# Janspiry/Image-Super-Resolution-via-Iterative-Refinement

Hardware: AMD Instinct MI355X
Metric: SR3 16->128 images/sec (2000-step sample) (higher is better)
Workload: dtype f32 via 3xbf16 split MFMA; 1 GPU; SR3 16->128 UNet (reference config/sr_sr3_16_128.json; BASELINE.json configs[1]), batch 16 per GPU, 2000-step p_sample_loop via hipGraph replay; step = one reverse step of the batch; images/s = n_gpus*batch/(2000*t_step); batch_per_gpu=16, global_batch=16, image_size=128, params=97807491, parallelism=independent batches per rank (no collective), weights=random init (PyTorch default, seed 0), output_finite=True

## Files before the change

image-super-resolution-via-iterative-refinement_amd/csrc/abi_ops.hip:

```cpp
#include "plan_internal.h"
#include "tile_code.h"

namespace {

enum Derive { DERIVE_IGEMM_WSPLIT, DERIVE_WINO, DERIVE_WINO_SPLIT };
size_t derive_bytes(const ConvParams& c, Derive kind) {
  const int Cin = c.C0 + c.C1;
  return (kind == DERIVE_IGEMM_WSPLIT ? igemm_wsplit_floats(c.Cout, c.ksize * c.ksize, Cin) : wino_weight_floats(c.Cout, Cin, kind == DERIVE_WINO_SPLIT)) * sizeof(float);
}
int derive_behind_slabs(const ConvParams& c, int tile, int ksplit, Derive kind, void* scratch, size_t* scratch_bytes, hipStream_t st, float** out) {
  const size_t slab = conv_splitk_bytes(c, tile, ksplit);
  const size_t need = derive_bytes(c, kind);
  if (!scratch || *scratch_bytes < slab + need) {
    set_error("conv: %s (%zu < %zu)", kind == DERIVE_IGEMM_WSPLIT ? "scratch too small for the pre-split weights" : "Winograd scratch too small", *scratch_bytes, slab + need);
    return SR3_E_NOMEM;
  }
  *out = reinterpret_cast<float*>(static_cast<char*>(scratch) + slab);
  *scratch_bytes = slab;
  const int Cin = c.C0 + c.C1;
  return kind == DERIVE_IGEMM_WSPLIT ? igemm_split_weights(c.w, c.Cout, c.ksize * c.ksize, Cin, *out, st)
                                     : wino_transform_weights(c.w, c.Cout, Cin, *out, st, kind == DERIVE_WINO_SPLIT);
}

int check_scratch_aligned(const void* scratch) {
// ... 205 lines not shown
  return attention_forward(qkv, B, N, C, out, static_cast<hipStream_t>(stream));
}
int sr3_attention_ex_f32(const float* qkv, int B, int N, int C, float* out, int split, void* stream) {
  if (!qkv || !out) { set_error("null argument"); return SR3_E_BADARG; }
  return attention_forward(qkv, B, N, C, out, static_cast<hipStream_t>(stream), split);
}
int sr3_film_embed_f32(int variant, int B, int inner, const float* level, const int64_t* timestep, const float* freq,
                       const float* w1, const float* b1, const float* w2, const float* b2, const float* wf,
                       const float* bf, int F, float* temb_scratch, float* film_out, void* stream) {
  EmbedParams e;
  memset(&e, 0, sizeof(e));
  e.variant = variant; e.B = B; e.inner = inner; e.level = level; e.tstep = timestep; e.freq = freq;
  e.w1 = w1; e.b1 = b1; e.w2 = w2; e.b2 = b2; e.wf = wf; e.bf = bf; e.F = F; e.temb = temb_scratch; e.film = film_out;
  return embed_forward(e, static_cast<hipStream_t>(stream));
}
int sr3_conv_in_f32(const float* a, int Ca, const float* b, int Cb, int B, int H, int W, const float* w,
                    const float* bias, int Cout, float* out, void* stream) {
  return conv_in_nchw(a, Ca, b, b ? Cb : 0, B, H, W, w, bias, Cout, out, nullptr, static_cast<hipStream_t>(stream));
}
int sr3_conv_out_f32(const float* x, const float* ss, int B, int H, int W, int C, const float* w, const float* bias,
                     int Cout, float* out, void* stream) {
  return conv_out_nchw(x, ss, B, H, W, C, w, bias, Cout, out, static_cast<hipStream_t>(stream));
}

}
```

image-super-resolution-via-iterative-refinement_amd/csrc/plan_abi.hip:

```cpp
#include <stdarg.h>
#include <stdlib.h>
#include <stdio.h>
#include <string.h>

#include <new>
#include <vector>

#include "plan_internal.h"
#include "tile_code.h"

namespace sr3 {

static thread_local char g_err[512] = "";
void set_error(const char* fmt, ...) {
  va_list ap;
  va_start(ap, fmt);
  vsnprintf(g_err, sizeof(g_err), fmt, ap);
  va_end(ap);
}
int hip_fail(hipError_t e, const char* what) {
  set_error("HIP error %d (%s) at %s", (int)e, hipGetErrorString(e), what);
  (void)hipGetLastError();
  return (int)e > 0 ? (int)e : 1;
}
const char* last_error() { return g_err; }

}

int check_store_wt(const sr3_plan*, const char*, int value) {
  if (value < 0 || value > STORE_WT_ALL) { set_error("store_wt %d: a mask of bits 0-2 (0 .. %d)", value, (int)STORE_WT_ALL); return SR3_E_BADARG; }
  return SR3_OK;
}
int check_gemm_epi(const sr3_plan*, const char*, int value) {
  if (value < 0 || value > 2) { set_error("gemm_epi %d: 0 (4-byte epilogue), 1 (16-byte stores) or 2 (16-byte stores written through L2)", value); return SR3_E_BADARG; }
  return SR3_OK;
}
int check_var_channels(const sr3_plan* plan, const char*, int value) {
  if (value != 0 && value * 2 != plan->out_ch) {
    set_error("var_channels %d: 0 or half of out_channel %d (the variance head of a learned-variance model)", value, plan->out_ch);
    return SR3_E_BADARG;
  }
  return SR3_OK;
}
// ... 316 lines not shown
```

image-super-resolution-via-iterative-refinement_amd/csrc/plan_internal.h:

```cpp
#pragma once
#include <map>
#include <string>
#include <vector>

#include "../../include/sr3_mi355x.h"
#include "sr3_common.h"

namespace sr3 {

struct Tensor {
  size_t off = 0;
  size_t bytes = 0;
  int C = 0, H = 0, W = 0;
  size_t stat_off = 0;
  int stat_T = 0;
  bool stats_done = false;
  bool valid = false;
};

struct ResLayer {
  std::string name;
  int cin, cout, skip;
  bool attn;
  int film_off;
// ... 137 lines not shown
  int wgrad_split = 1;
  int attn_split = 1;
  int attn_long = 0;
  int attn_heads = 1;
  int attn_head_dim = 0;
  int gemm_tile = 0;
  int gemm_split = 1;
  int gemm_wpre = 0;
  int fold_fuse = 1;
  int gemm2 = 1;
  int gemm_s2 = 1;
  int gemm_n64 = 1;
  int wino_ragged = 1;
  int wino_up = 1;
  int store_wt = 3;
  int gemm_epi = GEMM_EPI_DEFAULT;
  bool gemm_epi_named = false;
  int launch_gemm_epi() const { return gemm_epi_named ? gemm_epi : -1; }
  int train_geom = 0;
  int fork_side = 0;
  int loss_l2 = 0;
};

enum OptionEffect {
  OPT_FORWARD = 1,
  OPT_TRAIN = 2,
  OPT_REBUILD = OPT_FORWARD | OPT_TRAIN,
  OPT_STALE = 4,
  OPT_RELAY = 8,
  OPT_EXPERIMENT = 16,
};
typedef int (*OptionCheck)(const sr3_plan* plan, const char* key, int value);
int check_store_wt(const sr3_plan*, const char*, int);
int check_gemm_epi(const sr3_plan*, const char*, int);
int check_var_channels(const sr3_plan*, const char*, int);
int check_attn_heads(const sr3_plan*, const char*, int);
struct OptionRow { const char* name; int PlanOptions::*slot; unsigned effects; OptionCheck check; };
static const OptionRow PLAN_OPTIONS[] = {
  {"fuse_stats", &PlanOptions::fuse_stats, OPT_REBUILD, nullptr},
  {"tile_cfg", &PlanOptions::tile_cfg, OPT_REBUILD | OPT_STALE, nullptr},
  {"ksplit", &PlanOptions::ksplit, OPT_REBUILD, nullptr},
  {"keep_all", &PlanOptions::keep_all, OPT_REBUILD, nullptr},
  {"fuse_res", &PlanOptions::fuse_res, OPT_REBUILD, nullptr},
  {"split_bf16", &PlanOptions::split_bf16, OPT_REBUILD | OPT_STALE | OPT_EXPERIMENT, nullptr},
  {"winograd", &PlanOptions::winograd, OPT_REBUILD | OPT_STALE, nullptr},
  {"wino_split", &PlanOptions::wino_split, OPT_REBUILD | OPT_RELAY, nullptr},
  {"wino_split8", &PlanOptions::wino_split8, OPT_REBUILD, nullptr},
  {"wgrad_split", &PlanOptions::wgrad_split, 0, nullptr},
  {"attn_split", &PlanOptions::attn_split, 0, nullptr},
  {"store_wt", &PlanOptions::store_wt, 0, check_store_wt},
  {"gemm_epi", &PlanOptions::gemm_epi, 0, check_gemm_epi},
  {"attn_long", &PlanOptions::attn_long, OPT_REBUILD, nullptr},
  {"gemm_split", &PlanOptions::gemm_split, OPT_REBUILD | OPT_RELAY, nullptr},
  {"gemm_wpre", &PlanOptions::gemm_wpre, OPT_REBUILD | OPT_RELAY, nullptr},
  {"gemm2", &PlanOptions::gemm2, OPT_REBUILD | OPT_RELAY, nullptr},
  {"gemm_s2", &PlanOptions::gemm_s2, OPT_REBUILD | OPT_RELAY, nullptr},
  {"fork_side", &PlanOptions::fork_side, OPT_REBUILD, nullptr},
  {"gemm_n64", &PlanOptions::gemm_n64, OPT_REBUILD | OPT_RELAY, nullptr},
  {"fold_fuse", &PlanOptions::fold_fuse, OPT_REBUILD, nullptr},
  {"gemm_tile", &PlanOptions::gemm_tile, OPT_REBUILD, nullptr},
  {"wino2", &PlanOptions::wino2, OPT_REBUILD, nullptr},
  {"wino_ragged", &PlanOptions::wino_ragged, OPT_REBUILD, nullptr},
  {"wino_up", &PlanOptions::wino_up, OPT_REBUILD, nullptr},
  {"train_geom", &PlanOptions::train_geom, OPT_REBUILD, nullptr},
  {"loss_l2", &PlanOptions::loss_l2, 0, nullptr},
  {"var_channels", &PlanOptions::var_channels, OPT_REBUILD, check_var_channels},
// ... 99 lines not shown
```

image-super-resolution-via-iterative-refinement_amd/csrc/plan_run.hip:

```cpp
#include <string.h>

#include <vector>

#include "plan_internal.h"
#include "tile_code.h"

namespace sr3 {

template <typename T> static T* bind(char* base, size_t off) { return off == NO_OFF ? nullptr : reinterpret_cast<T*>(base + off); }
static const float* bind(const float* params, size_t off) { return off == NO_OFF ? nullptr : params + off; }

struct Bound {
  sr3_plan* P;
  const ForwardCall& f;
  const Regions& R;
  char* ws; char* stats; float* film;
  const float* params;
  hipStream_t st = nullptr;
  hipEvent_t mid = nullptr;
};

static FoldTail make_fold_tail(const FoldSpec& s, const Bound& b) {
  FoldTail f;
  memset(&f, 0, sizeof(f));
// ... 28 lines not shown
  }
  return SR3_OK;
}

static int launch_embed(const Op&, const Bound& b) {
  const sr3_plan* P = b.P;
  const ForwardCall& f = b.f;
  EmbedParams e;
  memset(&e, 0, sizeof(e));
  e.variant = P->d.variant; e.B = f.batch; e.inner = P->d.inner_channel;
  e.level = f.level; e.tstep = f.tstep; e.level_table = f.level_table; e.step_dev = f.step_dev; e.t_map = f.t_map; e.freq = f.freq;
  e.step_out = f.fuse ? const_cast<int*>(f.fuse->step_cur) : nullptr;
  e.w1 = b.params + P->emb_w1; e.b1 = b.params + P->emb_b1; e.w2 = b.params + P->emb_w2; e.b2 = b.params + P->emb_b2;
  e.wf = b.params + P->film_w; e.bf = b.params + P->film_b; e.F = P->film_rows();
  e.temb = reinterpret_cast<float*>(b.ws + b.R.temb_off); e.film = b.film;
  return embed_forward(e, b.st);
}

static int launch_conv_in(const Op& o, const Bound& b) {
  const Op::ConvIn& v = o.conv_in;
  const ForwardCall& f = b.f;
  const float* a0 = f.cond_channels > 0 ? f.cond : f.x;
  const int Ca = f.cond_channels > 0 ? f.cond_channels : v.x_channels;
  const float* a1 = f.cond_channels > 0 ? f.x : nullptr;
  const int Cb = f.cond_channels > 0 ? v.x_channels : 0;
  return conv_in_nchw(a0, Ca, a1, Cb, f.batch, v.H, v.W, b.params + v.w, b.params + v.bias, v.Cout, bind<float>(b.ws, v.out),
                      bind<double>(b.stats, v.ostat), b.st);
}

static int launch_stats(const Op& o, const Bound& b) {
  const Op::Stats& v = o.stats;
  if (o.fold_fused) {
    FoldTail ft = make_fold_tail(o.tail, b);
    return chan_stats_fold(bind<const float>(b.ws, v.src), b.f.batch, v.pixels, v.channels, bind<double>(b.stats, v.stat), ft, b.st);
  }
  return chan_stats(bind<const float>(b.ws, v.src), b.f.batch, v.pixels, v.channels, bind<double>(b.stats, v.stat), b.st);
}

static int launch_fold(const Op& o, const Bound& b) {
  const Op::Fold& v = o.fold;
  return gn_finalize(bind<const double>(b.stats, v.stat0), v.C0, v.T0, bind<const double>(b.stats, v.stat1), v.C1, v.T1, b.f.batch, v.pixels,
                     b.P->d.norm_groups, b.params + v.gamma, b.params + v.beta, 1e-5f, bind<float>(b.ws, b.R.ss_off + o.ss_rel), b.st,
// ... 31 lines not shown
  FoldTail ft;
  if (o.fold_fused) { ft = make_fold_tail(o.tail, b); c.fold = &ft; }
  return conv_forward(c, ch.tile_cfg, ch.ksplit, bind<float>(b.ws, b.R.scratch_off), b.R.scratch_bytes, b.st, b.mid);
}

static int launch_attn(const Op& o, const Bound& b) {
  const Op::Attn& v = o.attn;
  return attention_forward_heads(bind<const float>(b.ws, v.qkv), b.f.batch, v.tokens, v.channels, v.heads, bind<float>(b.ws, v.out), b.st,
                                 (b.P->opt.attn_split ? 1 : 0) | (v.tile_cfg == 24 ? 2 : 0));
}

static int launch_conv_out(const Op& o, const Bound& b) {
  const Op::ConvOut& v = o.conv_out;
  const int rows = (b.f.train || b.f.full_out) ? v.out_ch : v.out_ch - b.P->opt.var_channels;
  return conv_out_nchw(bind<const float>(b.ws, v.src), bind<const float>(b.ws, b.R.ss_off + o.ss_rel), b.f.batch, v.H, v.W, v.channels,
                       b.params + v.w, b.params + v.bias, rows, b.f.eps_out, b.st, b.f.fuse);
}

static int fork_op(sr3_plan* P, const Op& o, hipStream_t main_st, hipStream_t* st) {
  *st = main_st;
  if (o.wait_id >= 0 && o.wait_id < (int)P->join_ev.size()) SR3_HIP(hipStreamWaitEvent(main_st, P->join_ev[o.wait_id], 0));
  if (o.side_id < 0) return SR3_OK;
  if (!P->side_stream) SR3_HIP(hipStreamCreateWithFlags(&P->side_stream, hipStreamNonBlocking));
  while ((int)P->fork_ev.size() <= o.side_id) {
    hipEvent_t a, b;
    SR3_HIP(hipEventCreateWithFlags(&a, hipEventDisableTiming));
    SR3_HIP(hipEventCreateWithFlags(&b, hipEventDisableTiming));
    P->fork_ev.push_back(a); P->join_ev.push_back(b);
  }
  SR3_HIP(hipEventRecord(P->fork_ev[o.side_id], main_st));
  SR3_HIP(hipStreamWaitEvent(P->side_stream, P->fork_ev[o.side_id], 0));
// ... 90 lines not shown
```

image-super-resolution-via-iterative-refinement_amd/csrc/small_kernels.hip:

```cpp
#include <string.h>

#include <type_traits>

#include "conv_prologue.h"
#include "step_tail.h"

namespace sr3 {

__global__ __launch_bounds__(256) void k_chan_stats(const float* __restrict__ x, int HW, int C, int LQ,
                                                     int pix_per_block, double* __restrict__ stat) {
  __shared__ double red[256 * 8];
  const int tid = threadIdx.x;
  const int nq = C >> 2;
  const int ql = tid % LQ, pl = tid / LQ, PP = 256 / LQ;
  const int q = blockIdx.y * LQ + ql;
  const int b = blockIdx.z;
  const int T = gridDim.x;
  const int p0 = blockIdx.x * pix_per_block;
  const int p1 = min(HW, p0 + pix_per_block);
  double s[4] = {0, 0, 0, 0}, s2[4] = {0, 0, 0, 0};
  if (q < nq) {
    const float* base = x + (size_t)b * HW * C + q * 4;
    for (int p = p0 + pl; p < p1; p += PP) {
      const f32x4 v = *reinterpret_cast<const f32x4*>(base + (size_t)p * C);
// ... 428 lines not shown
    }
    const int co0 = cobase + cog * 16;
#pragma unroll
    for (int e4 = 0; e4 < 4; ++e4) {
      const int co = co0 + e4 * 4;
      if (co < Cout) {
        f32x4 o;
#pragma unroll
        for (int e = 0; e < 4; ++e) o[e] = acc[e4 * 4 + e] + (bias ? bias[co + e] : 0.f);
        *reinterpret_cast<f32x4*>(out + (size_t)m * Cout + co) = o;
      }
    }
  }
}

template <int CIN, int NB>
__global__ __launch_bounds__(256) void k_conv_in_mfma(const float* __restrict__ a, int Ca, const float* __restrict__ bsrc,
                                                       int Cb, int B, int H, int W, const float* __restrict__ w,
                                                       const float* __restrict__ bias, float* __restrict__ out,
                                                       double* __restrict__ ostat, int bpw, int T) {
  constexpr int K = 9 * CIN, KS = (K + 1) / 2, Cout = 32 * NB;
  const int lane = threadIdx.x & 63, wave = threadIdx.x >> 6;
  const int ln = lane & 31, h = lane >> 5;
  const int HW = H * W, bpi = HW >> 5;
  const int task = blockIdx.x * 4 + wave;
  if (task >= B * (bpi / bpw)) return;
  const int blk0 = task * bpw;
  const int b = blk0 / bpi;
  const int slice = (blk0 - b * bpi) / bpw;

  float bw[KS][NB], bn[NB];
#pragma unroll
  for (int s = 0; s < KS; ++s)
#pragma unroll
    for (int nb = 0; nb < NB; ++nb) {
      const int k = 2 * s + h;
      bw[s][nb] = k < K ? w[(size_t)(nb * 32 + ln) * K + k] : 0.f;
    }
#pragma unroll
  for (int nb = 0; nb < NB; ++nb) bn[nb] = bias ? bias[nb * 32 + ln] : 0.f;

  const float* plane[CIN];
#pragma unroll
  for (int c = 0; c < CIN; ++c)
    plane[c] = c < Ca ? a + ((size_t)b * Ca + c) * HW : bsrc + ((size_t)b * Cb + (c - Ca)) * HW;

  auto load_block = [&](int blk, float (&av)[KS]) {
    const int p0 = (blk - b * bpi) * 32;
    const int oh = p0 / W, ow = p0 - oh * W + ln;
    const int pixoff = oh * W + ow;
    const bool up = oh > 0, down = oh < H - 1, left = ow > 0, right = ow < W - 1;
#pragma unroll
// ... 65 lines not shown
static constexpr bool CONV_IN7_NB[5] = {false, true, true, true, true};
#endif
static int conv_in_bpw(int Cin, int H, int W, int Cout) {
  if ((Cin != 3 && Cin != 6 && Cin != 7 && Cin != 9) || (W & 31) || (Cout & 31) || Cout > 128 || Cout < 32) return 0;
  if (Cin == 9 && !CONV_IN9_NB[Cout / 32]) return 0;
  if (Cin == 7 && !CONV_IN7_NB[Cout / 32]) return 0;
  const int bpi = H * W / 32;
  return (bpi % 4 == 0) ? 4 : 1;
}
int conv_in_stat_slices(int Cin, int H, int W, int Cout) {
  const int bpw = conv_in_bpw(Cin, H, W, Cout);
  return bpw ? H * W / 32 / bpw : 0;
}

int conv_in_nchw(const float* a, int Ca, const float* b, int Cb, int B, int H, int W, const float* w,
                 const float* bias, int Cout, float* out, double* ostat, hipStream_t st) {
  if (const int bpw = conv_in_bpw(Ca + Cb, H, W, Cout)) {
    const int T = H * W / 32 / bpw;
    const long tasks = (long)B * T;
    const dim3 grid((unsigned)((tasks + 3) / 4));
#define SR3_CI(CIN, NB) hipLaunchKernelGGL((k_conv_in_mfma<CIN, NB>), grid, dim3(256), 0, st, a, Ca, b, Cb, B, H, W, w, bias, out, ostat, bpw, T)
#define SR3_CI_NB(CIN) do { if (nb == 1) SR3_CI(CIN, 1); else if (nb == 2) SR3_CI(CIN, 2); else if (nb == 3) SR3_CI(CIN, 3); else SR3_CI(CIN, 4); } while (0)
    const int nb = Cout / 32;
    switch (Ca + Cb) {
      case 3: SR3_CI_NB(3); break;
      case 6: SR3_CI_NB(6); break;
      case 7: SR3_CI_NB(7); break;
      default: SR3_CI_NB(9); break;
    }
#undef SR3_CI_NB
#undef SR3_CI
    SR3_LAUNCH_CHECK("k_conv_in_mfma");
    return SR3_OK;
  }
  if (ostat) { set_error("conv_in: fused output statistics need the MFMA form (W %% 32 == 0, Cout %% 32 == 0, 3, 6, 7 or 9 input channels)"); return SR3_E_UNSUPPORTED; }
  if (Cout & 3) { set_error("conv_in: Cout %% 4 != 0"); return SR3_E_UNSUPPORTED; }
  const int CoutP = (Cout + 63) & ~63;
  const size_t smem = (size_t)9 * (Ca + Cb) * CoutP * sizeof(float);
  if (smem > 64 * 1024) { set_error("conv_in: weights do not fit LDS (%zu B)", smem); return SR3_E_UNSUPPORTED; }
  const long M = (long)B * H * W;
  hipLaunchKernelGGL(k_conv_in_nchw, dim3((unsigned)((M + 63) / 64)), dim3(256), smem, st, a, Ca, b, Cb, B, H, W, w,
                     bias, Cout, out);
  SR3_LAUNCH_CHECK("k_conv_in_nchw");
  return SR3_OK;
}

#ifdef SR3_CONV_OUT_LINES
constexpr int OT_H = 8, OT_W = 32, OT_CK = 32, OT_LD = 36;
#else
constexpr int OT_H = 8, OT_W = 32, OT_CK = 16, OT_LD = 20;
#endif
constexpr int OT_Q = OT_CK / 4, OT_SUB = OT_CK / 16;
template <int COUT, bool FULL, bool FUSE, bool HIST>
__global__ __launch_bounds__(256) void k_conv_out_nchw(const float* __restrict__ x, const float* __restrict__ ss,
                                                        int B, int H, int W, int C, const float* __restrict__ w,
                                                        const float* __restrict__ bias, int Cout,
                                                        float* __restrict__ out, const StepFuse f) {
  __shared__ f32x4 tile_v[(OT_H + 2) * (OT_W + 2) * OT_LD / 4];
  float* tile = reinterpret_cast<float*>(tile_v);
  const int tid = threadIdx.x;
  const int tx = tid & 31, ty = tid >> 5;
  const int tiles_w = (W + OT_W - 1) / OT_W, tiles_h = (H + OT_H - 1) / OT_H;
  int bid = blockIdx.x;
  const int b = bid / (tiles_w * tiles_h);
  bid -= b * tiles_w * tiles_h;
  const int th = bid / tiles_w, tw = bid - th * tiles_w;
  const int h0 = th * OT_H, w0 = tw * OT_W;
  float acc[COUT <= 4 ? 4 : COUT] = {};
  constexpr int NPIX = (OT_H + 2) * (OT_W + 2);
  for (int c0 = 0; c0 < C; c0 += OT_CK) {
    __syncthreads();
    for (int i = tid; i < NPIX * OT_Q; i += 256) {
      const int pix = i / OT_Q, q = i % OT_Q;
      const int py = pix / (OT_W + 2), px = pix - py * (OT_W + 2);
      const int ih = h0 + py - 1, iw = w0 + px - 1;
      const int c = c0 + q * 4;
      f32x4 v = {0.f, 0.f, 0.f, 0.f};
      if (c < C && (unsigned)ih < (unsigned)H && (unsigned)iw < (unsigned)W) {
        v = *reinterpret_cast<const f32x4*>(x + (((size_t)b * H + ih) * W + iw) * C + c);
        const float* s = ss + ((size_t)b * C + c) * 2;
#pragma unroll
        for (int e = 0; e < 4; ++e) v[e] = silu_libm(fmaf(v[e], s[2 * e], s[2 * e + 1]));
      }
      *reinterpret_cast<f32x4*>(tile + pix * OT_LD + q * 4) = v;
    }
    __syncthreads();
#pragma unroll
    for (int sub = 0; sub < OT_SUB; ++sub) {
#pragma unroll
      for (int tap = 0; tap < 9; ++tap) {
        const float* tp = tile + ((ty + tap / 3) * (OT_W + 2) + tx + tap % 3) * OT_LD + sub * 16;
#pragma unroll
        for (int q = 0; q < 4; ++q) {
          if (FULL || c0 + sub * 16 + q * 4 < C) {
            const f32x4 v = *reinterpret_cast<const f32x4*>(tp + q * 4);
#pragma unroll
            for (int co = 0; co < COUT; ++co) {
              const float* wr = w + ((size_t)co * 9 + tap) * C + c0 + sub * 16 + q * 4;
              acc[co] = fmaf(v[0], wr[0], acc[co]);
              acc[co] = fmaf(v[1], wr[1], acc[co]);
              acc[co] = fmaf(v[2], wr[2], acc[co]);
// ... 17 lines not shown
      const size_t idx = (((size_t)b * Cout + co) * H + oh) * W + ow;
      const float e = acc[co] + (bias ? bias[co] : 0.f);
      if (!FUSE || out) out[idx] = e;
      if (FUSE) {
        const float xv = f.x[idx], zv = f.z ? f.z[idx] : 0.f;
        float hv = HIST ? f.hist[idx] : 0.f;
        const float xn = step_tail<HIST>(cf, f.clip, xv, e, zv, hv);
        if (HIST) f.hist[idx] = hv;
        f.x[idx] = xn;
      }
    }
  }
}

int conv_out_nchw(const float* x, const float* ss, int B, int H, int W, int C, const float* w, const float* bias,
                  int Cout, float* out_nchw, hipStream_t st, const StepFuse* fuse) {
  const bool wide = Cout == 6 || Cout == 8;
  if ((Cout > 4 && !wide) || Cout < 1) { set_error("conv_out: Cout %d > 4 unsupported", Cout); return SR3_E_UNSUPPORTED; }
  if (wide && fuse) { set_error("conv_out: no fused step tail on Cout %d (launch the prediction rows alone)", Cout); return SR3_E_UNSUPPORTED; }
  if (C & 3) { set_error("conv_out: C %% 4 != 0"); return SR3_E_UNSUPPORTED; }
  if (!fuse && !out_nchw) { set_error("conv_out: null output"); return SR3_E_BADARG; }
  const int tiles = ((W + OT_W - 1) / OT_W) * ((H + OT_H - 1) / OT_H) * B;
  StepFuse f;
  memset(&f, 0, sizeof(f));
  if (fuse) f = *fuse;
  if (const int rc = check_step_history("conv_out", f.c3, f.hist, f.x, out_nchw, (size_t)B * Cout * H * W * sizeof(float))) return rc;
  const bool hist = fuse && fuse->hist;
#define SR3_CO_LAUNCH3(N, FU, FS, HI)                                                                                        \
  hipLaunchKernelGGL((k_conv_out_nchw<N, FU, FS, HI>), dim3(tiles), dim3(256), 0, st, x, ss, B, H, W, C, w, bias, Cout, out_nchw, f);
#define SR3_CO_LAUNCH2(N, FU)                                                                                                \
  if (hist) { SR3_CO_LAUNCH3(N, FU, true, true) } else if (fuse) { SR3_CO_LAUNCH3(N, FU, true, false) } else { SR3_CO_LAUNCH3(N, FU, false, false) }
#define SR3_CO_LAUNCH(N)                                                                                                    \
  {                                                                                                                          \
    if (C % OT_CK == 0) { SR3_CO_LAUNCH2(N, true) } else { SR3_CO_LAUNCH2(N, false) }                                       \
  }
  switch (Cout) {
    case 1: SR3_CO_LAUNCH(1) break;
    case 2: SR3_CO_LAUNCH(2) break;
    case 3: SR3_CO_LAUNCH(3) break;
    case 4: SR3_CO_LAUNCH(4) break;
    case 6: if (C % OT_CK == 0) { SR3_CO_LAUNCH3(6, true, false, false) } else { SR3_CO_LAUNCH3(6, false, false, false) } break;
    default: if (C % OT_CK == 0) { SR3_CO_LAUNCH3(8, true, false, false) } else { SR3_CO_LAUNCH3(8, false, false, false) } break;
  }
#undef SR3_CO_LAUNCH
#undef SR3_CO_LAUNCH2
#undef SR3_CO_LAUNCH3
  SR3_LAUNCH_CHECK("k_conv_out_nchw");
  return SR3_OK;
}

__global__ __launch_bounds__(256) void k_embed(const EmbedParams p) {
  extern __shared__ f32x4 smem_v[];
  float* enc = reinterpret_cast<float*>(smem_v);
  float* hid = enc + p.inner;
  const int b = blockIdx.x, tid = threadIdx.x;
  const int half = p.inner / 2;
  float lv;
  if (p.variant == 0) {
    lv = p.step_dev ? p.level_table[p.step_dev[0] + 1] : p.level[b];
  } else {
    lv = p.step_dev ? (float)(p.t_map ? p.t_map[p.step_dev[0]] : p.step_dev[0]) : (float)p.tstep[b];
// ... 23 lines not shown

__global__ __launch_bounds__(256) void k_film(const EmbedParams p) {
  extern __shared__ f32x4 smem_v[];
  float* e = reinterpret_cast<float*>(smem_v);
  const int b = blockIdx.y;
  for (int k = threadIdx.x; k < p.inner; k += 256) e[k] = p.temb[(size_t)b * p.inner + k];
  __syncthreads();
  const int j = blockIdx.x * 256 + threadIdx.x;
  if (j >= p.F) return;
  float s = p.bf[j];
  const float* wr = p.wf + (size_t)j * p.inner;
  for (int k = 0; k < p.inner; ++k) s = fmaf(wr[k], e[k], s);
  p.film[(size_t)b * p.F + j] = s;
}

int embed_forward(const EmbedParams& p, hipStream_t st) {
  if (p.inner & 1) { set_error("embed: inner must be even"); return SR3_E_UNSUPPORTED; }
  hipLaunchKernelGGL(k_embed, dim3(p.B), dim3(256), (size_t)5 * p.inner * sizeof(float), st, p);
  SR3_LAUNCH_CHECK("k_embed");
  if (p.F > 0) {
    hipLaunchKernelGGL(k_film, dim3((p.F + 255) / 256, p.B), dim3(256), (size_t)p.inner * sizeof(float), st, p);
    SR3_LAUNCH_CHECK("k_film");
  }
  return SR3_OK;
}

template <bool CLIP, bool HIST, int V>
__global__ __launch_bounds__(256) void k_p_sample_update(float* __restrict__ x, const float* __restrict__ eps,
                                                          const float* __restrict__ z, StepTables tb,
                                                          const int* __restrict__ step_dev,
                                                          const int64_t* __restrict__ tps, int step_host,
                                                          int per_image, size_t total, const float* __restrict__ tc3,
// ... 70 lines not shown
```

image-super-resolution-via-iterative-refinement_amd/csrc/sr3_common.h:

```cpp
#pragma once
#include <hip/hip_runtime.h>
#include <stdint.h>
#include <stddef.h>

#include <atomic>

#include "../../include/sr3_mi355x.h"

namespace sr3 {

typedef float f32x4 __attribute__((ext_vector_type(4)));
typedef float f32x16 __attribute__((ext_vector_type(16)));

typedef __bf16 bf16x8 __attribute__((ext_vector_type(8)));
typedef __bf16 bf16x4 __attribute__((ext_vector_type(4)));

typedef __bf16 bf16x2 __attribute__((ext_vector_type(2)));

__device__ __forceinline__ void split3_pair(float x0, float x1, bf16x2& h, bf16x2& m, bf16x2& l) {
#ifdef SR3_SPLIT_NO_DOT2
  h[0] = (__bf16)x0; h[1] = (__bf16)x1;
  const float r0 = x0 - (float)h[0], r1 = x1 - (float)h[1];
  m[0] = (__bf16)r0; m[1] = (__bf16)r1;
  const float q0 = r0 - (float)m[0], q1 = r1 - (float)m[1];
// ... 219 lines not shown
size_t wino_weight_floats(int Cout, int Cin, bool split = false);
int wino_transform_weights(const float* w_ohwi, int Cout, int Cin, float* ufrag, hipStream_t st, bool split = false);
int conv3x3_wino_forward(const ConvParams& p, const float* ufrag, hipStream_t st);
bool wino2_fits(const ConvParams& p);
bool wino2_ragged_fits(const ConvParams& p);
int conv3x3_wino2_forward(const ConvParams& p, const WinoGeom& g, const float* ufrag, hipStream_t st);

int chan_stats_slices(int B, int HW, int C);
int chan_stats(const float* x, int B, int HW, int C, double* stat, hipStream_t st);
int gn_finalize(const double* stat0, int C0, int T0, const double* stat1, int C1, int T1, int B, int HW, int groups,
                const float* gamma, const float* beta, float eps, float* ss, hipStream_t st, float* mr = nullptr,
                const float* mod = nullptr, int mod_stride = 0);
int halo_stats_slices(const HaloGeom& g);
int conv_in_stat_slices(int Cin, int H, int W, int Cout);
int conv_in_nchw(const float* a, int Ca, const float* b, int Cb, int B, int H, int W, const float* w,
                 const float* bias, int Cout, float* out, double* ostat, hipStream_t st);
struct StepTables { const float* a; const float* b; const float* c1; const float* c2; const float* sigma; };

__device__ __forceinline__ float mul_rn(float a, float b) { float r = a * b; asm volatile("" : "+v"(r)); return r; }
__device__ __forceinline__ float add_rn(float a, float b) { float r = a + b; asm volatile("" : "+v"(r)); return r; }
__device__ __forceinline__ float sub_rn(float a, float b) { float r = a - b; asm volatile("" : "+v"(r)); return r; }
struct StepCoef { float a, b, c1, c2, c3, sigma; };
template <bool HIST>
__device__ __forceinline__ StepCoef load_step_coef(const StepTables& tb, const float* c3, int t) {
  return StepCoef{tb.a[t], tb.b[t], tb.c1[t], tb.c2[t], HIST ? c3[t] : 0.f, tb.sigma[t]};
}
__device__ __forceinline__ float step_x0(const StepCoef& k, bool clip, float x, float eps) {
  float x0 = sub_rn(mul_rn(k.a, x), mul_rn(k.b, eps));
  if (clip) x0 = fminf(fmaxf(x0, -1.f), 1.f);
  return x0;
}
// ... 23 lines not shown
  }
  return SR3_OK;
}

struct StepFuse {
  float* x;
  const float* z;
  StepTables tb;
  const int* step_cur;
  int* step_next;
  int clip;
  const float* c3;
  float* hist;
};
int conv_out_nchw(const float* x, const float* ss, int B, int H, int W, int C, const float* w,
                  const float* bias, int Cout, float* out_nchw, hipStream_t st, const StepFuse* fuse = nullptr);
struct EmbedParams {
  int variant;
  int B, inner;
  const float* level;
  const int64_t* tstep;
  const float* level_table;
  const int* step_dev;
  const int* t_map;
  int* step_out;
  const float* freq;
  const float* w1; const float* b1;
  const float* w2; const float* b2;
  const float* wf; const float* bf;
  int F;
  float* temb;
  float* film;
};
int embed_forward(const EmbedParams& p, hipStream_t st);
int attention_forward(const float* qkv, int B, int N, int C, float* out, hipStream_t st, int mode = 0);
bool attention_fits(int N, int C);
int attention_long_forward(const float* qkv, int B, int N, int C, float* out, hipStream_t st, bool split, int heads = 1);
int attention_forward_heads(const float* qkv, int B, int N, int C, int heads, float* out, hipStream_t st, int mode = 0);
int attention_forward_strided(const float* qkv, int B, int N, int C, int heads, float* out, hipStream_t st, int mode);
int attention_heads_check(const char* who, int C, int heads);
int p_sample_update(float* x, const float* eps, const float* z, StepTables tb, const int* step_dev,
                    const int64_t* t_per_sample, int step_host, int B, int per_image, hipStream_t st, bool clip = true,
                    const float* c3 = nullptr, float* hist = nullptr);
int step_decrement(int* step_dev, hipStream_t st);
int step_copy(int* step2, hipStream_t st);
int split3_selftest(int* bad_dev, hipStream_t st);
int q_sample(const float* x0, const float* z, const float* ca, const float* cb, int B, int per_image,
             float* out, hipStream_t st);

// ... 2 lines not shown
```

image-super-resolution-via-iterative-refinement_amd/sr3_hip/lib.py:

```python
import ctypes as C
import os

_HERE = os.path.dirname(os.path.abspath(__file__))
LIB_PATH = os.environ.get('SR3_LIBRARY') or os.path.join(_HERE, 'libsr3_mi355x.so')


class Sr3Error(RuntimeError):
    pass


class UnetDesc(C.Structure):
    _fields_ = [('variant', C.c_int), ('in_channel', C.c_int), ('out_channel', C.c_int),
                ('inner_channel', C.c_int), ('norm_groups', C.c_int), ('n_mults', C.c_int),
                ('channel_mults', C.c_int * 8), ('n_attn_res', C.c_int), ('attn_res', C.c_int * 8),
                ('res_blocks', C.c_int), ('image_size', C.c_int)]


class ParamInfo(C.Structure):
    _fields_ = [('name', C.c_char * 128), ('ndim', C.c_int), ('shape', C.c_int * 4), ('pack', C.c_int),
                ('offset', C.c_size_t), ('numel', C.c_size_t)]


class OpInfo(C.Structure):
    _fields_ = [('kind', C.c_int), ('tile_cfg', C.c_int), ('ksplit', C.c_int), ('ksize', C.c_int), ('stride', C.c_int),
# ... 129 lines not shown
                                           _P, _Z, _P, _P, _I, _P, _P]),
    'sr3_conv_dgrad_scratch_bytes': (_Z, [_P, _I, _I, _I, _I, _I, _I, _I, _I, C.POINTER(_Z), C.POINTER(_Z)]),
    'sr3_conv_dgrad_f32': (_I, [_P, _P, _P, _I, _I, _I, _I, _I, _I, _I, _I, _I, _P, _P, _Z, _P, _Z, _PI, _PI, _PI, _P]),
    'sr3_grad_route_f32': (_I, [_P, _I, _I, _I, _I, _I, _I, _P, _I, _P, _I, _P]),
    'sr3_colsums_scratch_bytes': (_Z, [_I, _I, _I]),
    'sr3_colsums_f32': (_I, [_P, _I, _I, _I, _P, _P, _I, _P, _Z, _P]),
    'sr3_embed_bwd_scratch_bytes': (_Z, [_I, _I]),
    'sr3_embed_bwd_f32': (_I, [_I, _I, _I, _I, _P, _P, _P, _P, _P, _P, _P, _P, _P, _P, _P, _P, _P, _P, _P, _P, _Z, _P]),
    'sr3_attention_f32': (_I, [_P, _I, _I, _I, _P, _P]),
    'sr3_attention_ex_f32': (_I, [_P, _I, _I, _I, _P, _I, _P]),
    'sr3_attention_heads_f32': (_I, [_P, _I, _I, _I, _I, _P, _I, _P]),
    'sr3_attention_bwd_heads_f32': (_I, [_P, _P, _P, _I, _I, _I, _I, _P, _P, _Z, _P]),
    'sr3_film_embed_f32': (_I, [_I, _I, _I, _P, _P, _P, _P, _P, _P, _P, _P, _P, _I, _P, _P, _P]),
    'sr3_conv_in_f32': (_I, [_P, _I, _P, _I, _I, _I, _I, _P, _P, _I, _P, _P]),
    'sr3_conv_out_f32': (_I, [_P, _P, _I, _I, _I, _I, _P, _P, _I, _P, _P]),
}

_lib = None


def load():
    global _lib
    if _lib is not None:
        return _lib
    if not os.path.exists(LIB_PATH):
        raise Sr3Error('libsr3_mi355x.so is not built (%s); run `python __graft_entry__.py build` '
                       'or csrc/build.sh -- there is no CPU / eager fallback' % LIB_PATH)
    lib = C.CDLL(LIB_PATH)
    for name, (res, args) in SIGNATURES.items():
        fn = getattr(lib, name)
# ... 24 lines not shown
```

include/sr3_mi355x.h:

```cpp
#ifndef SR3_MI355X_H
#define SR3_MI355X_H

#include <stddef.h>
#include <stdint.h>

#ifdef __cplusplus
extern "C" {
#endif

#define SR3_ABI_VERSION 1

#define SR3_E_BADARG (-1)
#define SR3_E_UNSUPPORTED (-2)
#define SR3_E_ALIGN (-3)
#define SR3_E_NOMEM (-4)
#define SR3_E_STATE (-5)

#define SR3_VARIANT_SR3 0
#define SR3_VARIANT_DDPM 1

typedef struct sr3_unet_desc {
  int variant;
  int in_channel, out_channel, inner_channel, norm_groups;
  int n_mults;
// ... 339 lines not shown

size_t sr3_embed_bwd_scratch_bytes(int B, int inner);
int sr3_embed_bwd_f32(int variant, int B, int inner, int F, const float* level, const int64_t* timestep, const float* freq,
                      const float* w1, const float* b1, const float* w2, const float* b2, const float* wf, const float* dfilm,
                      float* dw1, float* db1, float* dw2, float* db2, float* dwf, float* dbf, void* scratch, size_t scratch_bytes,
                      void* stream);

int sr3_film_embed_f32(int variant, int B, int inner, const float* level, const int64_t* timestep,
                       const float* freq, const float* w1, const float* b1, const float* w2, const float* b2,
                       const float* wf, const float* bf, int F, float* temb_scratch, float* film_out,
                       void* stream);
int sr3_conv_in_f32(const float* a_nchw, int Ca, const float* b_nchw, int Cb, int B, int H, int W,
                    const float* w_ohwi, const float* bias, int Cout, float* out_nhwc, void* stream);
int sr3_conv_out_f32(const float* x_nhwc, const float* ss, int B, int H, int W, int C, const float* w_ohwi,
                     const float* bias, int Cout, float* out_nchw, void* stream);

#ifdef __cplusplus
}
#endif
#endif
```

Before: 1.280 images/s.

## Add step-end kernel options: prefetched conv_out, LDS-staged conv_in filters, fused embed

Adds a step_ends option mask that selects three variants for the kernels at the ends of each UNet step. conv_out gains a register-prefetch path that loads the next channel chunk while the current one is computed, and it is on by default. conv_in can stage its filters in LDS, and the time embedding plus FiLM projection can run as a single launch; both of these are off by default. The prefetch path costs extra registers per thread, which may lower occupancy in a small tail kernel.

```diff
diff --git a/image-super-resolution-via-iterative-refinement_amd/csrc/abi_ops.hip b/image-super-resolution-via-iterative-refinement_amd/csrc/abi_ops.hip
--- a/image-super-resolution-via-iterative-refinement_amd/csrc/abi_ops.hip
+++ b/image-super-resolution-via-iterative-refinement_amd/csrc/abi_ops.hip
@@ -243,10 +243,29 @@
   e.w1 = w1; e.b1 = b1; e.w2 = w2; e.b2 = b2; e.wf = wf; e.bf = bf; e.F = F; e.temb = temb_scratch; e.film = film_out;
   return embed_forward(e, static_cast<hipStream_t>(stream));
 }
+int sr3_film_embed_ex_f32(int variant, int B, int inner, const float* level, const int64_t* timestep, const float* freq,
+                          const float* w1, const float* b1, const float* w2, const float* b2, const float* wf,
+                          const float* bf, int F, float* temb_scratch, float* film_out, int one_launch, void* stream) {
+  EmbedParams e;
+  memset(&e, 0, sizeof(e));
+  e.variant = variant; e.B = B; e.inner = inner; e.level = level; e.tstep = timestep; e.freq = freq;
+  e.w1 = w1; e.b1 = b1; e.w2 = w2; e.b2 = b2; e.wf = wf; e.bf = bf; e.F = F; e.temb = temb_scratch; e.film = film_out;
+  return embed_forward(e, static_cast<hipStream_t>(stream), one_launch != 0);
+}
 int sr3_conv_in_f32(const float* a, int Ca, const float* b, int Cb, int B, int H, int W, const float* w,
                     const float* bias, int Cout, float* out, void* stream) {
   return conv_in_nchw(a, Ca, b, b ? Cb : 0, B, H, W, w, bias, Cout, out, nullptr, static_cast<hipStream_t>(stream));
 }
+int sr3_conv_in_ex_f32(const float* a, int Ca, const float* b, int Cb, int B, int H, int W, const float* w,
+                       const float* bias, int Cout, float* out, double* stats, int lds_filters, void* stream) {
+  if (stats && !conv_in_stat_slices(Ca + (b ? Cb : 0), H, W, Cout)) { set_error("conv_in: no fused statistics at this shape (sr3_conv_in_stat_slices = 0)"); return SR3_E_UNSUPPORTED; }
+  return conv_in_nchw(a, Ca, b, b ? Cb : 0, B, H, W, w, bias, Cout, out, stats, static_cast<hipStream_t>(stream), lds_filters != 0);
+}
+int sr3_conv_in_stat_slices(int Cin, int H, int W, int Cout) { return conv_in_stat_slices(Cin, H, W, Cout); }
+int sr3_conv_out_ex_f32(const float* x, const float* ss, int B, int H, int W, int C, const float* w, const float* bias,
+                        int Cout, float* out, int prefetch, void* stream) {
+  return conv_out_nchw(x, ss, B, H, W, C, w, bias, Cout, out, static_cast<hipStream_t>(stream), nullptr, prefetch != 0);
+}
 int sr3_conv_out_f32(const float* x, const float* ss, int B, int H, int W, int C, const float* w, const float* bias,
                      int Cout, float* out, void* stream) {
   return conv_out_nchw(x, ss, B, H, W, C, w, bias, Cout, out, static_cast<hipStream_t>(stream));
diff --git a/image-super-resolution-via-iterative-refinement_amd/csrc/plan_abi.hip b/image-super-resolution-via-iterative-refinement_amd/csrc/plan_abi.hip
--- a/image-super-resolution-via-iterative-refinement_amd/csrc/plan_abi.hip
+++ b/image-super-resolution-via-iterative-refinement_amd/csrc/plan_abi.hip
@@ -27,6 +27,10 @@
 
 }
 
+int check_step_ends(const sr3_plan*, const char*, int value) {
+  if (value < 0 || value > STEP_ENDS_ALL) { set_error("step_ends %d: a mask of bits 0-2 (0 .. %d)", value, (int)STEP_ENDS_ALL); return SR3_E_BADARG; }
+  return SR3_OK;
+}
 int check_store_wt(const sr3_plan*, const char*, int value) {
   if (value < 0 || value > STORE_WT_ALL) { set_error("store_wt %d: a mask of bits 0-2 (0 .. %d)", value, (int)STORE_WT_ALL); return SR3_E_BADARG; }
   return SR3_OK;
diff --git a/image-super-resolution-via-iterative-refinement_amd/csrc/plan_internal.h b/image-super-resolution-via-iterative-refinement_amd/csrc/plan_internal.h
--- a/image-super-resolution-via-iterative-refinement_amd/csrc/plan_internal.h
+++ b/image-super-resolution-via-iterative-refinement_amd/csrc/plan_internal.h
@@ -175,6 +175,7 @@
   int wino_ragged = 1;
   int wino_up = 1;
   int store_wt = 3;
+  int step_ends = STEP_ENDS_DEFAULT;
   int gemm_epi = GEMM_EPI_DEFAULT;
   bool gemm_epi_named = false;
   int launch_gemm_epi() const { return gemm_epi_named ? gemm_epi : -1; }
@@ -194,6 +195,7 @@
 typedef int (*OptionCheck)(const sr3_plan* plan, const char* key, int value);
 int check_store_wt(const sr3_plan*, const char*, int);
 int check_gemm_epi(const sr3_plan*, const char*, int);
+int check_step_ends(const sr3_plan*, const char*, int);
 int check_var_channels(const sr3_plan*, const char*, int);
 int check_attn_heads(const sr3_plan*, const char*, int);
 struct OptionRow { const char* name; int PlanOptions::*slot; unsigned effects; OptionCheck check; };
@@ -211,6 +213,7 @@
   {"attn_split", &PlanOptions::attn_split, 0, nullptr},
   {"store_wt", &PlanOptions::store_wt, 0, check_store_wt},
   {"gemm_epi", &PlanOptions::gemm_epi, 0, check_gemm_epi},
+  {"step_ends", &PlanOptions::step_ends, 0, check_step_ends},
   {"attn_long", &PlanOptions::attn_long, OPT_REBUILD, nullptr},
   {"gemm_split", &PlanOptions::gemm_split, OPT_REBUILD | OPT_RELAY, nullptr},
   {"gemm_wpre", &PlanOptions::gemm_wpre, OPT_REBUILD | OPT_RELAY, nullptr},
diff --git a/image-super-resolution-via-iterative-refinement_amd/csrc/plan_run.hip b/image-super-resolution-via-iterative-refinement_amd/csrc/plan_run.hip
--- a/image-super-resolution-via-iterative-refinement_amd/csrc/plan_run.hip
+++ b/image-super-resolution-via-iterative-refinement_amd/csrc/plan_run.hip
@@ -66,7 +66,7 @@
   e.w1 = b.params + P->emb_w1; e.b1 = b.params + P->emb_b1; e.w2 = b.params + P->emb_w2; e.b2 = b.params + P->emb_b2;
   e.wf = b.params + P->film_w; e.bf = b.params + P->film_b; e.F = P->film_rows();
   e.temb = reinterpret_cast<float*>(b.ws + b.R.temb_off); e.film = b.film;
-  return embed_forward(e, b.st);
+  return embed_forward(e, b.st, (P->opt.step_ends & STEP_ENDS_EMBED) != 0);
 }
 
 static int launch_conv_in(const Op& o, const Bound& b) {
@@ -77,7 +77,7 @@
   const float* a1 = f.cond_channels > 0 ? f.x : nullptr;
   const int Cb = f.cond_channels > 0 ? v.x_channels : 0;
   return conv_in_nchw(a0, Ca, a1, Cb, f.batch, v.H, v.W, b.params + v.w, b.params + v.bias, v.Cout, bind<float>(b.ws, v.out),
-                      bind<double>(b.stats, v.ostat), b.st);
+                      bind<double>(b.stats, v.ostat), b.st, (b.P->opt.step_ends & STEP_ENDS_CONV_IN) != 0);
 }
 
 static int launch_stats(const Op& o, const Bound& b) {
@@ -139,7 +139,7 @@
   const Op::ConvOut& v = o.conv_out;
   const int rows = (b.f.train || b.f.full_out) ? v.out_ch : v.out_ch - b.P->opt.var_channels;
   return conv_out_nchw(bind<const float>(b.ws, v.src), bind<const float>(b.ws, b.R.ss_off + o.ss_rel), b.f.batch, v.H, v.W, v.channels,
-                       b.params + v.w, b.params + v.bias, rows, b.f.eps_out, b.st, b.f.fuse);
+                       b.params + v.w, b.params + v.bias, rows, b.f.eps_out, b.st, b.f.fuse, (b.P->opt.step_ends & STEP_ENDS_CONV_OUT) != 0);
 }
 
 static int fork_op(sr3_plan* P, const Op& o, hipStream_t main_st, hipStream_t* st) {
diff --git a/image-super-resolution-via-iterative-refinement_amd/csrc/small_kernels.hip b/image-super-resolution-via-iterative-refinement_amd/csrc/small_kernels.hip
--- a/image-super-resolution-via-iterative-refinement_amd/csrc/small_kernels.hip
+++ b/image-super-resolution-via-iterative-refinement_amd/csrc/small_kernels.hip
@@ -466,15 +466,21 @@
   }
 }
 
-template <int CIN, int NB>
+template <int CIN, int NB, bool LW>
 __global__ __launch_bounds__(256) void k_conv_in_mfma(const float* __restrict__ a, int Ca, const float* __restrict__ bsrc,
                                                        int Cb, int B, int H, int W, const float* __restrict__ w,
                                                        const float* __restrict__ bias, float* __restrict__ out,
                                                        double* __restrict__ ostat, int bpw, int T) {
   constexpr int K = 9 * CIN, KS = (K + 1) / 2, Cout = 32 * NB;
+  constexpr int KP = K | 1;
+  __shared__ float wl[LW ? Cout * KP + 1 : 1];
   const int lane = threadIdx.x & 63, wave = threadIdx.x >> 6;
   const int ln = lane & 31, h = lane >> 5;
   const int HW = H * W, bpi = HW >> 5;
+  if (LW) {
+    for (int i = threadIdx.x; i < Cout * K; i += 256) wl[(i / K) * KP + i % K] = w[i];
+    __syncthreads();
+  }
   const int task = blockIdx.x * 4 + wave;
   if (task >= B * (bpi / bpw)) return;
   const int blk0 = task * bpw;
@@ -487,7 +493,8 @@
 #pragma unroll
     for (int nb = 0; nb < NB; ++nb) {
       const int k = 2 * s + h;
-      bw[s][nb] = k < K ? w[(size_t)(nb * 32 + ln) * K + k] : 0.f;
+      if (LW) bw[s][nb] = k < K ? wl[(nb * 32 + ln) * KP + k] : 0.f;
+      else bw[s][nb] = k < K ? w[(size_t)(nb * 32 + ln) * K + k] : 0.f;
     }
 #pragma unroll
   for (int nb = 0; nb < NB; ++nb) bn[nb] = bias ? bias[nb * 32 + ln] : 0.f;
@@ -583,12 +590,13 @@
 }
 
 int conv_in_nchw(const float* a, int Ca, const float* b, int Cb, int B, int H, int W, const float* w,
-                 const float* bias, int Cout, float* out, double* ostat, hipStream_t st) {
+                 const float* bias, int Cout, float* out, double* ostat, hipStream_t st, bool lds_filters) {
   if (const int bpw = conv_in_bpw(Ca + Cb, H, W, Cout)) {
     const int T = H * W / 32 / bpw;
     const long tasks = (long)B * T;
     const dim3 grid((unsigned)((tasks + 3) / 4));
-#define SR3_CI(CIN, NB) hipLaunchKernelGGL((k_conv_in_mfma<CIN, NB>), grid, dim3(256), 0, st, a, Ca, b, Cb, B, H, W, w, bias, out, ostat, bpw, T)
+#define SR3_CI_LW(CIN, NB, LW) hipLaunchKernelGGL((k_conv_in_mfma<CIN, NB, LW>), grid, dim3(256), 0, st, a, Ca, b, Cb, B, H, W, w, bias, out, ostat, bpw, T)
+#define SR3_CI(CIN, NB) do { if (lds_filters) SR3_CI_LW(CIN, NB, true); else SR3_CI_LW(CIN, NB, false); } while (0)
 #define SR3_CI_NB(CIN) do { if (nb == 1) SR3_CI(CIN, 1); else if (nb == 2) SR3_CI(CIN, 2); else if (nb == 3) SR3_CI(CIN, 3); else SR3_CI(CIN, 4); } while (0)
     const int nb = Cout / 32;
     switch (Ca + Cb) {
@@ -599,6 +607,7 @@
     }
 #undef SR3_CI_NB
 #undef SR3_CI
+#undef SR3_CI_LW
     SR3_LAUNCH_CHECK("k_conv_in_mfma");
     return SR3_OK;
   }
@@ -620,7 +629,7 @@
 constexpr int OT_H = 8, OT_W = 32, OT_CK = 16, OT_LD = 20;
 #endif
 constexpr int OT_Q = OT_CK / 4, OT_SUB = OT_CK / 16;
-template <int COUT, bool FULL, bool FUSE, bool HIST>
+template <int COUT, bool FULL, bool FUSE, bool HIST, bool PF>
 __global__ __launch_bounds__(256) void k_conv_out_nchw(const float* __restrict__ x, const float* __restrict__ ss,
                                                         int B, int H, int W, int C, const float* __restrict__ w,
                                                         const float* __restrict__ bias, int Cout,
@@ -637,23 +646,69 @@
   const int h0 = th * OT_H, w0 = tw * OT_W;
   float acc[COUT <= 4 ? 4 : COUT] = {};
   constexpr int NPIX = (OT_H + 2) * (OT_W + 2);
+  constexpr int OT_NIT = (NPIX * OT_Q + 255) / 256;
+  static_assert(256 % OT_Q == 0, "a thread stages one quad of channels");
+  const int pq = tid % OT_Q;
+  unsigned poff[PF ? OT_NIT : 1] = {};
+  unsigned inb = 0;
+  f32x4 pv[PF ? OT_NIT : 1] = {};
+  float ps[8] = {};
+  const float* xb = x + (size_t)b * H * W * C;
+  const float* sb = ss + (size_t)b * C * 2;
+  auto fetch = [&](int c0) {
+    const unsigned c = FULL ? c0 + pq * 4 : min(c0 + pq * 4, C - 4);
+#pragma unroll
+    for (int it = 0; it < OT_NIT; ++it) pv[it] = *reinterpret_cast<const f32x4*>(xb + (poff[it] + c));
+#pragma unroll
+    for (int e = 0; e < 8; ++e) ps[e] = sb[2 * c + e];
+  };
+  if (PF) {
+#pragma unroll
+    for (int it = 0; it < OT_NIT; ++it) {
+      const int i = tid + it * 256;
+      const int pix = i / OT_Q;
+      const int py = pix / (OT_W + 2), px = pix - py * (OT_W + 2);
+      const int ih = h0 + py - 1, iw = w0 + px - 1;
+      if (i < NPIX * OT_Q && (unsigned)ih < (unsigned)H && (unsigned)iw < (unsigned)W) {
+        poff[it] = (unsigned)((ih * W + iw) * C);
+        inb |= 1u << it;
+      }
+    }
+    fetch(0);
+  }
   for (int c0 = 0; c0 < C; c0 += OT_CK) {
     __syncthreads();
-    for (int i = tid; i < NPIX * OT_Q; i += 256) {
-      const int pix = i / OT_Q, q = i % OT_Q;
-      const int py = pix / (OT_W + 2), px = pix - py * (OT_W + 2);
-      const int ih = h0 + py - 1, iw = w0 + px - 1;
-      const int c = c0 + q * 4;
-      f32x4 v = {0.f, 0.f, 0.f, 0.f};
-      if (c < C && (unsigned)ih < (unsigned)H && (unsigned)iw < (unsigned)W) {
-        v = *reinterpret_cast<const f32x4*>(x + (((size_t)b * H + ih) * W + iw) * C + c);
-        const float* s = ss + ((size_t)b * C + c) * 2;
-#pragma unroll
-        for (int e = 0; e < 4; ++e) v[e] = silu_libm(fmaf(v[e], s[2 * e], s[2 * e + 1]));
-      }
-      *reinterpret_cast<f32x4*>(tile + pix * OT_LD + q * 4) = v;
+    if (PF) {
+      const bool cin = FULL || c0 + pq * 4 < C;
+#pragma unroll
+      for (int it = 0; it < OT_NIT; ++it) {
+        const int i = tid + it * 256;
+        if (i < NPIX * OT_Q) {
+          const bool staged = cin && ((inb >> it) & 1);
+          f32x4 v;
+#pragma unroll
+          for (int e = 0; e < 4; ++e) v[e] = staged ? silu_libm(fmaf(pv[it][e], ps[2 * e], ps[2 * e + 1])) : 0.f;
+          *reinterpret_cast<f32x4*>(tile + (i / OT_Q) * OT_LD + pq * 4) = v;
+        }
+      }
+    } else {
+      for (int i = tid; i < NPIX * OT_Q; i += 256) {
+        const int pix = i / OT_Q, q = i % OT_Q;
+        const int py = pix / (OT_W + 2), px = pix - py * (OT_W + 2);
+        const int ih = h0 + py - 1, iw = w0 + px - 1;
+        const int c = c0 + q * 4;
+        f32x4 v = {0.f, 0.f, 0.f, 0.f};
+        if (c < C && (unsigned)ih < (unsigned)H && (unsigned)iw < (unsigned)W) {
+          v = *reinterpret_cast<const f32x4*>(x + (((size_t)b * H + ih) * W + iw) * C + c);
+          const float* s = ss + ((size_t)b * C + c) * 2;
+#pragma unroll
+          for (int e = 0; e < 4; ++e) v[e] = silu_libm(fmaf(v[e], s[2 * e], s[2 * e + 1]));
+        }
+        *reinterpret_cast<f32x4*>(tile + pix * OT_LD + q * 4) = v;
+      }
     }
     __syncthreads();
+    if (PF && c0 + OT_CK < C) fetch(c0 + OT_CK);
 #pragma unroll
     for (int sub = 0; sub < OT_SUB; ++sub) {
 #pragma unroll
@@ -701,7 +756,7 @@
 }
 
 int conv_out_nchw(const float* x, const float* ss, int B, int H, int W, int C, const float* w, const float* bias,
-                  int Cout, float* out_nchw, hipStream_t st, const StepFuse* fuse) {
+                  int Cout, float* out_nchw, hipStream_t st, const StepFuse* fuse, bool prefetch) {
   const bool wide = Cout == 6 || Cout == 8;
   if ((Cout > 4 && !wide) || Cout < 1) { set_error("conv_out: Cout %d > 4 unsupported", Cout); return SR3_E_UNSUPPORTED; }
   if (wide && fuse) { set_error("conv_out: no fused step tail on Cout %d (launch the prediction rows alone)", Cout); return SR3_E_UNSUPPORTED; }
@@ -713,8 +768,11 @@
   if (fuse) f = *fuse;
   if (const int rc = check_step_history("conv_out", f.c3, f.hist, f.x, out_nchw, (size_t)B * Cout * H * W * sizeof(float))) return rc;
   const bool hist = fuse && fuse->hist;
+  const bool pf = prefetch && (long long)H * W * C < (1ll << 31);
+#define SR3_CO_LAUNCH4(N, FU, FS, HI, PF)                                                                                    \
+  hipLaunchKernelGGL((k_conv_out_nchw<N, FU, FS, HI, PF>), dim3(tiles), dim3(256), 0, st, x, ss, B, H, W, C, w, bias, Cout, out_nchw, f);
 #define SR3_CO_LAUNCH3(N, FU, FS, HI)                                                                                        \
-  hipLaunchKernelGGL((k_conv_out_nchw<N, FU, FS, HI>), dim3(tiles), dim3(256), 0, st, x, ss, B, H, W, C, w, bias, Cout, out_nchw, f);
+  if (pf) { SR3_CO_LAUNCH4(N, FU, FS, HI, true) } else { SR3_CO_LAUNCH4(N, FU, FS, HI, false) }
 #define SR3_CO_LAUNCH2(N, FU)                                                                                                \
   if (hist) { SR3_CO_LAUNCH3(N, FU, true, true) } else if (fuse) { SR3_CO_LAUNCH3(N, FU, true, false) } else { SR3_CO_LAUNCH3(N, FU, false, false) }
 #define SR3_CO_LAUNCH(N)                                                                                                    \
@@ -732,6 +790,7 @@
 #undef SR3_CO_LAUNCH
 #undef SR3_CO_LAUNCH2
 #undef SR3_CO_LAUNCH3
+#undef SR3_CO_LAUNCH4
   SR3_LAUNCH_CHECK("k_conv_out_nchw");
   return SR3_OK;
 }
@@ -785,8 +844,115 @@
   p.film[(size_t)b * p.F + j] = s;
 }
 
-int embed_forward(const EmbedParams& p, hipStream_t st) {
+constexpr int EF_INNER = 64, EF_R = EF_INNER * EF_INNER / 64, EF_NI = 4;
+__global__ __launch_bounds__(256) void k_embed_film(const EmbedParams p, int sh) {
+  extern __shared__ f32x4 smem_v[];
+  const int inner = 1 << sh, hdim = 4 * inner, n = inner * hdim;
+  float* enc = reinterpret_cast<float*>(smem_v);
+  float* hid = enc + EF_NI * inner;
+  float* emb = hid + EF_NI * hdim;
+  float* tile = emb + EF_NI * inner;
+  const int b0 = blockIdx.y * EF_NI, tid = threadIdx.x;
+  const int j0 = blockIdx.x * 256;
+  const int nf = min(256, p.F - j0) * inner;
+  const float* wfr = p.wf + (size_t)j0 * inner;
+  float r2[EF_R], rf[EF_R];
+#pragma unroll
+  for (int it = 0; it < EF_R; ++it) {
+    const int i = tid + it * 256;
+    r2[it] = i < n ? p.w2[i] : 0.f;
+    rf[it] = i < nf ? wfr[i] : 0.f;
+  }
+#pragma unroll
+  for (int it = 0; it < EF_R; ++it) {
+    const int i = tid + it * 256;
+    if (i < n) tile[(i >> sh) * (inner + 1) + (i & (inner - 1))] = p.w1[i];
+  }
+  const int half = inner / 2;
+  if (p.step_out && blockIdx.y == 0 && blockIdx.x == 0 && tid == 0) p.step_out[0] = p.step_dev[0];
+  for (int i = tid; i < EF_NI * half; i += 256) {
+    const int m = i >> (sh - 1), k = i & (half - 1);
+    const int b = min(b0 + m, p.B - 1);
+    float lv;
+    if (p.variant == 0) {
+      lv = p.step_dev ? p.level_table[p.step_dev[0] + 1] : p.level[b];
+    } else {
+      lv = p.step_dev ? (float)(p.t_map ? p.t_map[p.step_dev[0]] : p.step_dev[0]) : (float)p.tstep[b];
+    }
+    const float arg = lv * p.freq[k];
+    enc[m * inner + k] = sinf(arg);
+    enc[m * inner + half + k] = cosf(arg);
+  }
+  __syncthreads();
+  if (tid < hdim) {
+    float s[EF_NI];
+#pragma unroll
+    for (int m = 0; m < EF_NI; ++m) s[m] = p.b1[tid];
+    const float* wr = tile + tid * (inner + 1);
+#pragma unroll 8
+    for (int k = 0; k < inner; ++k) {
+      const float wv = wr[k];
+#pragma unroll
+      for (int m = 0; m < EF_NI; ++m) s[m] = fmaf(wv, enc[m * inner + k], s[m]);
+    }
+#pragma unroll
+    for (int m = 0; m < EF_NI; ++m) hid[m * hdim + tid] = silu_libm(s[m]);
+  }
+  __syncthreads();
+#pragma unroll
+  for (int it = 0; it < EF_R; ++it) {
+    const int i = tid + it * 256;
+    if (i < n) tile[(i >> (sh + 2)) * (hdim + 1) + (i & (hdim - 1))] = r2[it];
+  }
+  __syncthreads();
+  if (tid < EF_NI * inner) {
+    const int m = tid >> sh, j = tid & (inner - 1);
+    float s = p.b2[j];
+    const float* wr = tile + j * (hdim + 1);
+    const float* hv = hid + m * hdim;
+#pragma unroll 8
+    for (int k = 0; k < hdim; ++k) s = fmaf(wr[k], hv[k], s);
+    s = (p.variant == 1) ? silu_libm(s) : s;
+    emb[tid] = s;
+    if (blockIdx.x == 0 && b0 + m < p.B) p.temb[(size_t)(b0 + m) * inner + j] = s;
+  }
+  __syncthreads();
+#pragma unroll
+  for (int it = 0; it < EF_R; ++it) {
+    const int i = tid + it * 256;
+    if (i < nf) tile[(i >> sh) * (inner + 1) + (i & (inner - 1))] = rf[it];
+  }
+  __syncthreads();
+  const int j = j0 + tid;
+  if (j >= p.F) return;
+  float s[EF_NI];
+#pragma unroll
+  for (int m = 0; m < EF_NI; ++m) s[m] = p.bf[j];
+  const float* wr = tile + tid * (inner + 1);
+#pragma unroll 8
+  for (int k = 0; k < inner; ++k) {
+    const float wv = wr[k];
+#pragma unroll
+    for (int m = 0; m < EF_NI; ++m) s[m] = fmaf(wv, emb[m * inner + k], s[m]);
+  }
+#pragma unroll
+  for (int m = 0; m < EF_NI; ++m)
+    if (b0 + m < p.B) p.film[(size_t)(b0 + m) * p.F + j] = s[m];
+}
+
+int embed_forward(const EmbedParams& p, hipStream_t st, bool one_launch) {
   if (p.inner & 1) { set_error("embed: inner must be even"); return SR3_E_UNSUPPORTED; }
+  if (one_launch && p.inner >= 8 && p.inner <= EF_INNER && (p.inner & (p.inner - 1)) == 0) {
+    int sh = 0;
+    while ((1 << sh) < p.inner) ++sh;
+    const int bytes = (EF_NI * 6 * p.inner + 256 * (p.inner + 1)) * (int)sizeof(float);
+    static std::atomic<uint64_t> done{0};
+    constexpr int max_bytes = (EF_NI * 6 * EF_INNER + 256 * (EF_INNER + 1)) * (int)sizeof(float);
+    if (const int rc = ensure_max_lds(reinterpret_cast<const void*>(k_embed_film), max_bytes, done)) return rc;
+    hipLaunchKernelGGL(k_embed_film, dim3(p.F > 0 ? (p.F + 255) / 256 : 1, (p.B + EF_NI - 1) / EF_NI), dim3(256), (size_t)bytes, st, p, sh);
+    SR3_LAUNCH_CHECK("k_embed_film");
+    return SR3_OK;
+  }
   hipLaunchKernelGGL(k_embed, dim3(p.B), dim3(256), (size_t)5 * p.inner * sizeof(float), st, p);
   SR3_LAUNCH_CHECK("k_embed");
   if (p.F > 0) {
diff --git a/image-super-resolution-via-iterative-refinement_amd/csrc/sr3_common.h b/image-super-resolution-via-iterative-refinement_amd/csrc/sr3_common.h
--- a/image-super-resolution-via-iterative-refinement_amd/csrc/sr3_common.h
+++ b/image-super-resolution-via-iterative-refinement_amd/csrc/sr3_common.h
@@ -257,7 +257,14 @@
 int halo_stats_slices(const HaloGeom& g);
 int conv_in_stat_slices(int Cin, int H, int W, int Cout);
 int conv_in_nchw(const float* a, int Ca, const float* b, int Cb, int B, int H, int W, const float* w,
-                 const float* bias, int Cout, float* out, double* ostat, hipStream_t st);
+                 const float* bias, int Cout, float* out, double* ostat, hipStream_t st, bool lds_filters = false);
+enum {
+  STEP_ENDS_EMBED = 1,
+  STEP_ENDS_CONV_IN = 2,
+  STEP_ENDS_CONV_OUT = 4,
+  STEP_ENDS_ALL = 7,
+  STEP_ENDS_DEFAULT = STEP_ENDS_CONV_OUT,
+};
 struct StepTables { const float* a; const float* b; const float* c1; const float* c2; const float* sigma; };
 
 __device__ __forceinline__ float mul_rn(float a, float b) { float r = a * b; asm volatile("" : "+v"(r)); return r; }
@@ -311,7 +318,7 @@
   float* hist;
 };
 int conv_out_nchw(const float* x, const float* ss, int B, int H, int W, int C, const float* w,
-                  const float* bias, int Cout, float* out_nchw, hipStream_t st, const StepFuse* fuse = nullptr);
+                  const float* bias, int Cout, float* out_nchw, hipStream_t st, const StepFuse* fuse = nullptr, bool prefetch = true);
 struct EmbedParams {
   int variant;
   int B, inner;
@@ -329,7 +336,7 @@
   float* temb;
   float* film;
 };
-int embed_forward(const EmbedParams& p, hipStream_t st);
+int embed_forward(const EmbedParams& p, hipStream_t st, bool one_launch = false);
 int attention_forward(const float* qkv, int B, int N, int C, float* out, hipStream_t st, int mode = 0);
 bool attention_fits(int N, int C);
 int attention_long_forward(const float* qkv, int B, int N, int C, float* out, hipStream_t st, bool split, int heads = 1);
diff --git a/image-super-resolution-via-iterative-refinement_amd/sr3_hip/lib.py b/image-super-resolution-via-iterative-refinement_amd/sr3_hip/lib.py
--- a/image-super-resolution-via-iterative-refinement_amd/sr3_hip/lib.py
+++ b/image-super-resolution-via-iterative-refinement_amd/sr3_hip/lib.py
@@ -167,6 +167,10 @@
     'sr3_film_embed_f32': (_I, [_I, _I, _I, _P, _P, _P, _P, _P, _P, _P, _P, _P, _I, _P, _P, _P]),
     'sr3_conv_in_f32': (_I, [_P, _I, _P, _I, _I, _I, _I, _P, _P, _I, _P, _P]),
     'sr3_conv_out_f32': (_I, [_P, _P, _I, _I, _I, _I, _P, _P, _I, _P, _P]),
+    'sr3_film_embed_ex_f32': (_I, [_I, _I, _I, _P, _P, _P, _P, _P, _P, _P, _P, _P, _I, _P, _P, _I, _P]),
+    'sr3_conv_in_ex_f32': (_I, [_P, _I, _P, _I, _I, _I, _I, _P, _P, _I, _P, _P, _I, _P]),
+    'sr3_conv_in_stat_slices': (_I, [_I, _I, _I, _I]),
+    'sr3_conv_out_ex_f32': (_I, [_P, _P, _I, _I, _I, _I, _P, _P, _I, _P, _I, _P]),
 }
 
 _lib = None
diff --git a/include/sr3_mi355x.h b/include/sr3_mi355x.h
--- a/include/sr3_mi355x.h
+++ b/include/sr3_mi355x.h
@@ -377,6 +377,15 @@
                     const float* w_ohwi, const float* bias, int Cout, float* out_nhwc, void* stream);
 int sr3_conv_out_f32(const float* x_nhwc, const float* ss, int B, int H, int W, int C, const float* w_ohwi,
                      const float* bias, int Cout, float* out_nchw, void* stream);
+int sr3_film_embed_ex_f32(int variant, int B, int inner, const float* level, const int64_t* timestep,
+                          const float* freq, const float* w1, const float* b1, const float* w2, const float* b2,
+                          const float* wf, const float* bf, int F, float* temb_scratch, float* film_out,
+                          int one_launch, void* stream);
+int sr3_conv_in_stat_slices(int Cin, int H, int W, int Cout);
+int sr3_conv_in_ex_f32(const float* a_nchw, int Ca, const float* b_nchw, int Cb, int B, int H, int W,
+                       const float* w_ohwi, const float* bias, int Cout, float* out_nhwc, double* stats, int lds_filters, void* stream);
+int sr3_conv_out_ex_f32(const float* x_nhwc, const float* ss, int B, int H, int W, int C, const float* w_ohwi,
+                        const float* bias, int Cout, float* out_nchw, int prefetch, void* stream);
 
 #ifdef __cplusplus
 }
```

New measurement: 1.281 images/s, median of 6. No clear change (+0.1%).
